# florasion/D-VQVAE

Measured on AMD Instinct MI355X. Metric: grasps/sec at batch=65536, N=1024 pts, K=512, higher is better.
Workload: dtype f32 (GEMMs: every fp32 operand as two fp16 pieces, a1 = fp16(a), a2 = fp16((a - a1) * 2^11), weights pre-scaled by one power of two per output row; the 3 partial products a1 b1, a1 b2, a2 b1 are exact in fp32 and accumulate in TWO fp32 accumulators (large / cross terms) on v_mfma_f32_16x16x32_f16; d

## Files before the change

d-vqvae_amd/csrc/gemm_f16x2.hip:

```cpp
#include "dvq_internal.h"
#include "gemm_common.h"

namespace {

typedef _Float16 h8 __attribute__((ext_vector_type(8)));
typedef _Float16 h2 __attribute__((ext_vector_type(2)));
typedef float f32x2 __attribute__((ext_vector_type(2)));

constexpr int TM = 128, TN = 256, BK = 32;
constexpr int A_PL = TM * 64;
constexpr int W_PL = TN * 64;
constexpr int STAGE = 2 * A_PL + 2 * W_PL;
constexpr float LO_SCALE = 1.0f / 2048.0f;

__device__ __forceinline__ int swz16(int row) { return (4 - ((row >> 2) & 3)) & 3; }

__device__ __forceinline__ void split2(const f32x4& lo, const f32x4& hi, h8& p1, h8& p2) {
    unsigned hb[4], lb[4];
    const float m2048 = -2048.0f;
#pragma unroll
    for (int j = 0; j < 4; ++j) {
        const float a0 = j < 2 ? lo[2 * j] : hi[2 * j - 4], a1 = j < 2 ? lo[2 * j + 1] : hi[2 * j - 3];
        hb[j] = __builtin_bit_cast(unsigned, __builtin_convertvector(f32x2{a0, a1}, h2));
        const float t0 = a0 * 2048.0f, t1 = a1 * 2048.0f;
        asm("v_fma_mixlo_f16 %0, %1, %2, %3 op_sel:[0,0,0] op_sel_hi:[1,0,0]" : "=v"(lb[j]) : "v"(hb[j]), "v"(m2048), "v"(t0));
        asm("v_fma_mixhi_f16 %0, %1, %2, %3 op_sel:[1,0,0] op_sel_hi:[1,0,0]" : "+v"(lb[j]) : "v"(hb[j]), "v"(m2048), "v"(t1));
    }
    p1 = __builtin_bit_cast(h8, uint4{hb[0], hb[1], hb[2], hb[3]});
    p2 = __builtin_bit_cast(h8, uint4{lb[0], lb[1], lb[2], lb[3]});
}

__device__ __forceinline__ f32x4 f16x2_combine(const f32x4& hi, const f32x4& lo, const float* ws, int n, bool vec) {
    f32x4 v = hi + lo * LO_SCALE;
    if (vec) v *= *reinterpret_cast<const f32x4*>(ws + n);
    return v;
}

__device__ __forceinline__ float relu_nan(float x) { return x < 0.f ? 0.f : x; }

template <int EPI>
__device__ __forceinline__ void f16x2_store_block(const GemmParams& p, long m, int n, f32x4 v, bool full) {
    if (full) {
        if (p.bias) v += *reinterpret_cast<const f32x4*>(p.bias + n);
        if constexpr (EPI == EPI_RESID) v += *reinterpret_cast<const f32x4*>(p.resid + m * p.ldr + n);
        if (p.relu) { v[0] = relu_nan(v[0]); v[1] = relu_nan(v[1]); v[2] = relu_nan(v[2]); v[3] = relu_nan(v[3]); }
        *reinterpret_cast<f32x4*>(p.out + m * p.ldo + n) = v;
    } else {
#pragma unroll
        for (int c = 0; c < 4; ++c) {
            if (n + c >= p.N) continue;
            float x = v[c] * p.wscale[n + c] + (p.bias ? p.bias[n + c] : 0.f);
            if constexpr (EPI == EPI_RESID) x += p.resid[m * p.ldr + n + c];
            if (p.relu) x = relu_nan(x);
            p.out[m * p.ldo + n + c] = x;
        }
    }
}

__device__ __forceinline__ float gate_act(float a, float g) {
    const float th = fmaf(-2.0f, __builtin_amdgcn_rcpf(1.0f + __builtin_amdgcn_exp2f(2.8853900817779268f * a)), 1.0f);
    const float sg = __builtin_amdgcn_rcpf(1.0f + __builtin_amdgcn_exp2f(-1.4426950408889634f * g));
    return th * sg;
}

__device__ __forceinline__ void f16x2_store_gate(const GemmParams& p, long m, int na, int c, f32x4 a, f32x4 g, const float* crow) {
    const int nb = na + 32;
    if (p.bias) {
        a += *reinterpret_cast<const f32x4*>(p.bias + na);
        g += *reinterpret_cast<const f32x4*>(p.bias + nb);
    }
    if (p.pre) {
        *reinterpret_cast<f32x4*>(p.pre + m * p.ldpre + na) = a;
        *reinterpret_cast<f32x4*>(p.pre + m * p.ldpre + nb) = g;
    }
    if (crow) {
        a += *reinterpret_cast<const f32x4*>(crow + na);
        g += *reinterpret_cast<const f32x4*>(crow + nb);
    }
    f32x4 o;
#pragma unroll
    for (int q = 0; q < 4; ++q) o[q] = gate_act(a[q], g[q]);
    *reinterpret_cast<f32x4*>(p.out + m * p.ldo + c) = o;
}

__device__ __forceinline__ f32x4 ld4(const float* q) { return *reinterpret_cast<const f32x4*>(q); }
__device__ __forceinline__ void st4(float* q, const f32x4& v) { *reinterpret_cast<f32x4*>(q) = v; }

template <int EPI, int NJ>
__device__ __forceinline__ void f16x2_epilogue_inside(const GemmParams& p, f32x4 (&hi)[NJ][4], f32x4 (&lo)[NJ][4], long m0w, int n0w, int c0w,
                                                      int lane) {
    static_assert(EPI == EPI_BIAS || EPI == EPI_RESID || (EPI == EPI_GATE && NJ == 4), "store epilogues with operands");
    const long m = m0w + (lane & 15);
    const int l4 = 4 * (lane >> 4), nl = n0w + l4;
    f32x4 ws[NJ], bq[NJ], aq[NJ][4];
    const float* crow[4];
#pragma unroll
    for (int jn = 0; jn < NJ; ++jn) ws[jn] = ld4(p.wscale + nl + 16 * jn);
    if (p.bias) {
#pragma unroll
        for (int jn = 0; jn < NJ; ++jn) bq[jn] = ld4(p.bias + nl + 16 * jn);
    }
    if constexpr (EPI == EPI_GATE) {
        if (p.cls) {
#pragma unroll
            for (int i = 0; i < 4; ++i) crow[i] = p.cls + (long)p.label[m + 16 * i] * p.N + nl;
        }
    }
#pragma unroll
    for (int jn = 0; jn < NJ; ++jn)
#pragma unroll
        for (int i = 0; i < 4; ++i) hi[jn][i] = hi[jn][i] + lo[jn][i] * LO_SCALE;
    if constexpr (EPI == EPI_RESID) {
#pragma unroll
        for (int i = 0; i < 4; ++i)
#pragma unroll
            for (int jn = 0; jn < NJ; ++jn) aq[jn][i] = ld4(p.resid + (m + 16 * i) * p.ldr + nl + 16 * jn);
    } else if constexpr (EPI == EPI_GATE) {
        if (p.cls) {
#pragma unroll
            for (int i = 0; i < 4; ++i)
#pragma unroll
                for (int jn = 0; jn < NJ; ++jn) aq[jn][i] = ld4(crow[i] + 16 * jn);
        }
    }
#pragma unroll
    for (int i = 0; i < 4; ++i) {
        if constexpr (EPI == EPI_GATE) {
#pragma unroll
            for (int jn = 0; jn < 2; ++jn) {
                f32x4 a = hi[jn][i] * ws[jn], g = hi[jn + 2][i] * ws[jn + 2];
                if (p.bias) { a += bq[jn]; g += bq[jn + 2]; }
                if (p.pre) {
                    st4(p.pre + (m + 16 * i) * p.ldpre + nl + 16 * jn, a);
                    st4(p.pre + (m + 16 * i) * p.ldpre + nl + 16 * jn + 32, g);
                }
                if (p.cls) { a += aq[jn][i]; g += aq[jn + 2][i]; }
                f32x4 o;
#pragma unroll
                for (int q = 0; q < 4; ++q) o[q] = gate_act(a[q], g[q]);
                st4(p.out + (m + 16 * i) * p.ldo + c0w + l4 + 16 * jn, o);
            }
        } else {
#pragma unroll
            for (int jn = 0; jn < NJ; ++jn) {
                f32x4 v = hi[jn][i] * ws[jn];
                if (p.bias) v += bq[jn];
                if constexpr (EPI == EPI_RESID) v += aq[jn][i];
                if (p.relu) { v[0] = relu_nan(v[0]); v[1] = relu_nan(v[1]); v[2] = relu_nan(v[2]); v[3] = relu_nan(v[3]); }
                st4(p.out + (m + 16 * i) * p.ldo + nl + 16 * jn, v);
            }
        }
    }
}

template <int NJ, bool INIT>
__device__ __forceinline__ void f16x2_init_acc(const GemmParams& p, f32x4 (&hi)[NJ][4], f32x4 (&lo)[NJ][4], long m0w, int n0w, int lane) {
    if constexpr (!INIT) {
#pragma unroll
        for (int a = 0; a < NJ; ++a)
#pragma unroll
            for (int c = 0; c < 4; ++c) { hi[a][c] = f32x4{0.f, 0.f, 0.f, 0.f}; lo[a][c] = f32x4{0.f, 0.f, 0.f, 0.f}; }
        return;
    }
    const int lr = lane & 15, lc = lane >> 4;
    if (p.acc_hi && m0w + 64 <= p.M && n0w + 16 * NJ <= p.N) {
        long r[4];
#pragma unroll
        for (int i = 0; i < 4; ++i) r[i] = m0w + i * 16 + lr;
        if (p.acc_row) {
#pragma unroll
            for (int i = 0; i < 4; ++i) r[i] = p.acc_row[r[i]];
        }
#pragma unroll
        for (int i = 0; i < 4; ++i)
#pragma unroll
            for (int jn = 0; jn < NJ; ++jn) {
                hi[jn][i] = ld4(p.acc_hi + r[i] * p.ldacc + n0w + jn * 16 + 4 * lc);
                lo[jn][i] = ld4(p.acc_lo + r[i] * p.ldacc + n0w + jn * 16 + 4 * lc);
            }
        return;
    }
#pragma unroll
    for (int i = 0; i < 4; ++i) {
        const long m = m0w + i * 16 + lr;
        const bool row_ok = p.acc_hi && m < p.M;
        const long r = row_ok ? (p.acc_row ? p.acc_row[m] : m) : 0;
#pragma unroll
        for (int jn = 0; jn < NJ; ++jn) {
            const int n = n0w + jn * 16 + 4 * lc;
            if (row_ok && n < p.N) {
                hi[jn][i] = *reinterpret_cast<const f32x4*>(p.acc_hi + r * p.ldacc + n);
                lo[jn][i] = *reinterpret_cast<const f32x4*>(p.acc_lo + r * p.ldacc + n);
            } else {
                hi[jn][i] = f32x4{0.f, 0.f, 0.f, 0.f};
                lo[jn][i] = f32x4{0.f, 0.f, 0.f, 0.f};
            }
        }
    }
}

template <int EPI, int NJ = 4>
__device__ __forceinline__ void f16x2_epilogue(const GemmParams& p, f32x4 (&hi)[NJ][4], f32x4 (&lo)[NJ][4], long m0w, int n0w, int c0w,
                                               int lane) {
    static_assert(NJ == 4 || EPI != EPI_GATE, "the gate pairs a wave's tanh columns with their partners 32 columns further");
    if constexpr (EPI == EPI_BIAS || EPI == EPI_RESID || (EPI == EPI_GATE && NJ == 4)) {
        const bool vec_ok = EPI == EPI_GATE || ((p.N % 4 == 0) && (p.ldo % 4 == 0) && (EPI != EPI_RESID || p.ldr % 4 == 0));
        if (vec_ok && m0w + 64 <= p.M && n0w + 16 * NJ <= p.N) {
            f16x2_epilogue_inside<EPI, NJ>(p, hi, lo, m0w, n0w, c0w, lane);
            return;
        }
    }
    const int lr = lane & 15, lc = lane >> 4;
#pragma unroll
    for (int i = 0; i < 4; ++i) {
        const long m = m0w + i * 16 + lr;
        if (m >= p.M) continue;
        if constexpr (EPI == EPI_BIAS || EPI == EPI_RESID) {
            const bool vec_ok = (p.N % 4 == 0) && (p.ldo % 4 == 0) && (EPI != EPI_RESID || p.ldr % 4 == 0);
#pragma unroll
            for (int jn = 0; jn < NJ; ++jn) {
                const int n = n0w + jn * 16 + 4 * lc;
                if (n >= p.N) continue;
                const bool full = vec_ok && n + 3 < p.N;
                f16x2_store_block<EPI>(p, m, n, f16x2_combine(hi[jn][i], lo[jn][i], p.wscale, n, full), full);
            }
        } else if constexpr (EPI == EPI_STATE) {
#pragma unroll
            for (int jn = 0; jn < NJ; ++jn) {
                const int n = n0w + jn * 16 + 4 * lc;
                if (n >= p.N) continue;
                *reinterpret_cast<f32x4*>(p.out + m * p.ldo + n) = hi[jn][i];
                *reinterpret_cast<f32x4*>(p.pre + m * p.ldpre + n) = lo[jn][i];
            }
        } else if constexpr (EPI == EPI_GATE) {
            if constexpr (NJ == 4) {
            if (n0w >= p.N) continue;
            const float* crow = p.cls ? p.cls + (long)p.label[m] * p.N : nullptr;
#pragma unroll
            for (int jn = 0; jn < 2; ++jn) {
                const int nl = jn * 16 + 4 * lc;
                const int na = n0w + nl;
                f16x2_store_gate(p, m, na, c0w + nl, f16x2_combine(hi[jn][i], lo[jn][i], p.wscale, na, true),
                                 f16x2_combine(hi[jn + 2][i], lo[jn + 2][i], p.wscale, na + 32, true), crow);
            }
            }
        }
    }
}

constexpr int PP_STAGES = 3;
constexpr size_t PP_SMEM = PP_STAGES * STAGE;
constexpr size_t PP_SMEM_N128 = PP_STAGES * (2 * A_PL + 2 * 128 * 64);

struct PpCursorA {
    int s, k_left;
    const float* a_ptr;
    __device__ __forceinline__ void open(const GemmParams& p, int src_i, long m0, int tid) {
        s = src_i;
        if (s >= p.nsrc) { k_left = 0; return; }
        const GemmSrc& src = p.src[s];
        k_left = src.K;
        long m = m0 + (tid >> 2);
        if (m >= p.M) m = p.M - 1;
        if (src.arow) m = src.arow[m];
        a_ptr = src.A + m * src.lda + 8 * (tid & 3);
    }
    __device__ __forceinline__ bool valid() const { return k_left > 0; }
    __device__ __forceinline__ void advance(const GemmParams& p, long m0, int tid) {
        a_ptr += BK;
        k_left -= BK;
        if (k_left <= 0) open(p, s + 1, m0, tid);
    }
};

template <int NJ>
struct PpCursorW {
    int s, k_left;
    const uint16_t* w_ptr[NJ];
    __device__ __forceinline__ void open(const GemmParams& p, int src_i, int n0, int wave, int lane) {
        s = src_i;
        if (s >= p.nsrc) { k_left = 0; return; }
        const GemmSrc& src = p.src[s];
        k_left = src.K;
#pragma unroll
        for (int i = 0; i < NJ; ++i) {
            const int id = wave * NJ + i;
            const int pl = id / (4 * NJ), rb = id % (4 * NJ);
            const int row = rb * 16 + (lane >> 2);
            int n = n0 + row;
            if (n >= p.N) n = p.N - 1;
            w_ptr[i] = src.Wp + pl * src.wp_plane + (long)n * src.ldw + 8 * ((lane & 3) ^ swz16(row));
        }
    }
    __device__ __forceinline__ void issue(char* stage, int wave) const {
#pragma unroll
        for (int i = 0; i < NJ; ++i) {
            const int id = wave * NJ + i;
            const int pl = id / (4 * NJ), rb = id % (4 * NJ);
            __builtin_amdgcn_global_load_lds((const __attribute__((address_space(1))) void*)w_ptr[i],
                                             (__attribute__((address_space(3))) void*)(stage + 2 * A_PL + pl * (64 * NJ * 64) + rb * 1024), 16, 0, 0);
        }
    }
    __device__ __forceinline__ void advance(const GemmParams& p, int n0, int wave, int lane) {
#pragma unroll
        for (int i = 0; i < NJ; ++i) w_ptr[i] += BK;
        k_left -= BK;
        if (k_left <= 0) open(p, s + 1, n0, wave, lane);
    }
};

template <int EPI, int NJ, bool INIT>
__global__ __launch_bounds__(512, 1) void gemm_f16x2_pp_kernel(const GemmParams p, int T) {
    extern __shared__ __attribute__((aligned(16))) char smem_c[];
    constexpr int TN = 64 * NJ, W_PL = TN * 64, STAGE = 2 * A_PL + 2 * W_PL;
    const int tid = threadIdx.x;
    const int tiles_n = (p.N + TN - 1) / TN;
    const long tiles_m = (p.M + TM - 1) / TM;
    const long b = blockIdx.x;
    const long j = b >> 3;
    const long mt = (j / tiles_n) * 8 + (b & 7);
    const int nt = (int)(j % tiles_n);
    if (mt >= tiles_m) return;
    const long m0 = mt * TM;
    const int n0 = nt * TN;
    const int lane = tid & 63;
    const int wave = __builtin_amdgcn_readfirstlane(tid >> 6);
    const int wm = wave >> 2, wn = wave & 3;

    PpCursorA ca;
    PpCursorW<NJ> cw;
    cw.open(p, 0, n0, wave, lane);
    const int a_dst = (tid >> 2) * 64 + 16 * ((tid & 3) ^ swz16(tid >> 2));
    f32x4 alo, ahi;
    auto load_a = [&](f32x4& qlo, f32x4& qhi) {
        qlo = *reinterpret_cast<const f32x4*>(ca.a_ptr);
        qhi = *reinterpret_cast<const f32x4*>(ca.a_ptr + 4);
        ca.advance(p, m0, tid);
    };
    auto store_a = [&](char* stage, const f32x4& qlo, const f32x4& qhi) {
        h8 p1, p2;
        split2(qlo, qhi, p1, p2);
        *reinterpret_cast<h8*>(stage + a_dst) = p1;
        *reinterpret_cast<h8*>(stage + A_PL + a_dst) = p2;
    };
    cw.issue(smem_c, wave);
    cw.advance(p, n0, wave, lane);
    if (T > 1) {
        cw.issue(smem_c + STAGE, wave);
        cw.advance(p, n0, wave, lane);
    }
    ca.open(p, 0, m0, tid);
    f32x4 a0lo, a0hi, a1lo, a1hi;
    load_a(a0lo, a0hi);
    if (T > 1) load_a(a1lo, a1hi);
    if (T > 2) load_a(alo, ahi);
    store_a(smem_c, a0lo, a0hi);
    if (T > 1) store_a(smem_c + STAGE, a1lo, a1hi);
    asm volatile("s_waitcnt vmcnt(0) lgkmcnt(0)" ::: "memory");
    __builtin_amdgcn_s_barrier();

    f32x4 hi[NJ][4], lo[NJ][4];
    f16x2_init_acc<NJ, INIT>(p, hi, lo, m0 + wm * 64, n0 + wn * 16 * NJ, lane);

    const int rd = (lane & 15) * 64 + 16 * ((lane >> 4) ^ swz16(lane & 15));
    if (wave >= 4) __builtin_amdgcn_s_barrier();
    int cur_st = 0, nx_st = 2;
    for (int t = 0; t < T; ++t) {
        const char* st = smem_c + cur_st * STAGE;
        h8 af[4][2], wf[NJ][2];
#pragma unroll
        for (int i = 0; i < 4; ++i)
#pragma unroll
            for (int pl = 0; pl < 2; ++pl) {
                if (DVQ_DIAG_ON && (p.dbg_abl & 128)) {
                    af[i][pl] = h8{};
                    if (i < NJ) wf[i][pl] = h8{};
                    continue;
                }
                if (DVQ_DIAG_ON && (p.dbg_abl & 64) && pl == 1) {
                    af[i][1] = af[i][0];
                    if (i < NJ) wf[i][1] = wf[i][0];
                    continue;
                }
                af[i][pl] = *reinterpret_cast<const h8*>(st + pl * A_PL + (wm * 64 + i * 16) * 64 + rd);
                if (i < NJ) wf[i][pl] = *reinterpret_cast<const h8*>(st + 2 * A_PL + pl * W_PL + (wn * 16 * NJ + i * 16) * 64 + rd);
            }
        asm volatile("s_waitcnt vmcnt(0)" ::: "memory");
        if (t + 2 < T) {
            char* nx = smem_c + nx_st * STAGE;
            if (!(DVQ_DIAG_ON && (p.dbg_abl & 16))) store_a(nx, alo, ahi);
            if (!(DVQ_DIAG_ON && (p.dbg_abl & 8))) cw.issue(nx, wave);
            cw.advance(p, n0, wave, lane);
            if (t + 3 < T && !(DVQ_DIAG_ON && (p.dbg_abl & 32))) load_a(alo, ahi);
        }
        asm volatile("s_waitcnt lgkmcnt(0)" ::: "memory");
        __builtin_amdgcn_s_barrier();
        __builtin_amdgcn_s_setprio(1);
        if (DVQ_DIAG_ON && (p.dbg_abl & 2)) {
#pragma unroll
            for (int i = 0; i < 4; ++i) asm volatile("" : : "v"(af[i][0]), "v"(af[i][1]), "v"(wf[i < NJ ? i : 0][0]), "v"(wf[i < NJ ? i : 0][1]));
        } else {
#pragma unroll
        for (int jn = 0; jn < NJ; ++jn)
#pragma unroll
            for (int i = 0; i < 4; ++i) hi[jn][i] = __builtin_amdgcn_mfma_f32_16x16x32_f16(wf[jn][0], af[i][0], hi[jn][i], 0, 0, 0);
#pragma unroll
        for (int jn = 0; jn < NJ; ++jn)
#pragma unroll
            for (int i = 0; i < 4; ++i) lo[jn][i] = __builtin_amdgcn_mfma_f32_16x16x32_f16(wf[jn][1], af[i][0], lo[jn][i], 0, 0, 0);
#pragma unroll
        for (int jn = 0; jn < NJ; ++jn)
#pragma unroll
            for (int i = 0; i < 4; ++i) lo[jn][i] = __builtin_amdgcn_mfma_f32_16x16x32_f16(wf[jn][0], af[i][1], lo[jn][i], 0, 0, 0);
        }
        __builtin_amdgcn_s_setprio(0);
        if (!(DVQ_DIAG_ON && (p.dbg_abl & 512))) __builtin_amdgcn_s_barrier();
        cur_st = cur_st == PP_STAGES - 1 ? 0 : cur_st + 1;
        nx_st = nx_st == PP_STAGES - 1 ? 0 : nx_st + 1;
    }
    if (wave < 4) __builtin_amdgcn_s_barrier();
    if (DVQ_DIAG_ON && (p.dbg_abl & 256)) {
        if (hi[0][0][0] + lo[0][0][0] == 12345.678f) p.out[0] = 1.f;
        return;
    }
    f16x2_epilogue<EPI, NJ>(p, hi, lo, m0 + wm * 64, n0 + wn * 16 * NJ, (n0 >> 1) + wn * 32, lane);
}

template <int EPI, int NJ, bool INIT>
int launch_pp(const GemmParams& p, hipStream_t stream) {
    constexpr size_t smem = NJ == 4 ? PP_SMEM : PP_SMEM_N128;
    static DvqOncePerDevice attr_once;
    DVQ_PROPAGATE(dvq_lds_limit(attr_once, reinterpret_cast<const void*>(&gemm_f16x2_pp_kernel<EPI, NJ, INIT>), smem, "gemm_f16x2"));
    const long grid = gemm_padded_grid((p.M + TM - 1) / TM, (p.N + 64 * NJ - 1) / (64 * NJ));
    const double ksum = gemm_ksum(p);
    {
        DVQ_PROF(gemm_prof_name(EPI, p.prof_cls), 2.0 * (double)p.M * p.N * ksum, ((double)p.M + p.N) * ksum * 4, stream);
        DVQ_LAUNCH((gemm_f16x2_pp_kernel<EPI, NJ, INIT>), dim3((unsigned)grid), dim3(512), smem, stream, p, gemm_ktiles(p, BK));
    }
    DVQ_CHECK_LAUNCH("gemm_f16x2");
    return DVQ_OK;
}

template <int EPI, bool INIT = false>
int launch_tiled(const GemmParams& p, hipStream_t stream) {
    if constexpr (EPI != EPI_GATE) {
        const long tiles_m = (p.M + TM - 1) / TM, tiles_n = (p.N + TN - 1) / TN, tiles_n2 = (p.N + 127) / 128, cus = dvq_num_cus();
        const long r256 = (tiles_m * tiles_n + cus - 1) / cus, r128 = (tiles_m * tiles_n2 + cus - 1) / cus;
        bool narrow = r128 < 2 * r256;
        if (dvq_knobs().gemm_tn == 128) narrow = true;
        if (dvq_knobs().gemm_tn == 256) narrow = false;
        if (narrow) return launch_pp<EPI, 2, INIT>(p, stream);
    }
    return launch_pp<EPI, 4, INIT>(p, stream);
}

template <int NB>
struct SkinnySlot {
    uint4 w[NB][2];
    f32x4 a[2];
};

template <int NB>
struct SkinnyCursor16 {
    int s, k_left;
    const float* a_ptr;
    const uint16_t* w_ptr[NB][2];

    __device__ __forceinline__ void open(const GemmParams& p, int src_i, long m, const int (&n)[NB], int lc) {
        s = src_i;
        const GemmSrc& src = p.src[s];
        k_left = src.K;
        a_ptr = src.A + (src.arow ? src.arow[m] : m) * src.lda + 8 * lc;
#pragma unroll
        for (int b = 0; b < NB; ++b)
#pragma unroll
            for (int pl = 0; pl < 2; ++pl) w_ptr[b][pl] = src.Wp + pl * src.wp_plane + (long)n[b] * src.ldw + 8 * lc;
    }
    __device__ __forceinline__ void load(SkinnySlot<NB>& t) const {
#pragma unroll
        for (int b = 0; b < NB; ++b) {
            t.w[b][0] = *reinterpret_cast<const uint4*>(w_ptr[b][0]);
            t.w[b][1] = *reinterpret_cast<const uint4*>(w_ptr[b][1]);
        }
        t.a[0] = *reinterpret_cast<const f32x4*>(a_ptr);
        t.a[1] = *reinterpret_cast<const f32x4*>(a_ptr + 4);
    }
    __device__ __forceinline__ void advance(const GemmParams& p, long m, const int (&n)[NB], int lc, bool last) {
        if (last) return;
        k_left -= BK;
        if (k_left > 0) {
            a_ptr += BK;
#pragma unroll
            for (int b = 0; b < NB; ++b) { w_ptr[b][0] += BK; w_ptr[b][1] += BK; }
        } else open(p, s + 1, m, n, lc);
    }
};

template <int EPI, int R>
__device__ __forceinline__ int skinny_col(int g, int j) {
    if constexpr (EPI == EPI_GATE) {
        constexpr int per64 = 32 / R;
        const int c0 = 64 * (g / per64) + R * (g % per64);
        return j < R ? c0 + j : (j < 2 * R ? c0 + 32 + (j - R) : c0);
    } else {
        return j < R ? R * g + j : R * g;
    }
}

template <int EPI, int R, int NB, int PF>
__device__ __forceinline__ void skinny_body(const GemmParams& p, int T, int groups) {
    const int lane = threadIdx.x;
    const int lr = lane & 15, lc = lane >> 4;
    const long mb0 = (long)blockIdx.y * 16;
    long m = mb0 + lr;
    if (m >= p.M) m = p.M - 1;
    int g[NB], n[NB];
#pragma unroll
    for (int b = 0; b < NB; ++b) {
        g[b] = (int)blockIdx.x * NB + b;
        if (g[b] >= groups) g[b] = groups - 1;
        n[b] = skinny_col<EPI, R>(g[b], lr);
        if (n[b] >= p.N) n[b] = p.N - 1;
    }
    f32x4 hi[NB], lo[NB];
#pragma unroll
    for (int b = 0; b < NB; ++b) {
        hi[b] = f32x4{0.f, 0.f, 0.f, 0.f};
        lo[b] = f32x4{0.f, 0.f, 0.f, 0.f};
        const int nc0 = skinny_col<EPI, R>(g[b], 4 * lc);
        const bool col_live = EPI == EPI_GATE ? 4 * lc < 2 * R : (4 * lc < R && nc0 < p.N);
        if (p.acc_hi && col_live && mb0 + lr < p.M) {
            const long r = p.acc_row ? p.acc_row[mb0 + lr] : mb0 + lr;
            hi[b] = *reinterpret_cast<const f32x4*>(p.acc_hi + r * p.ldacc + nc0);
            lo[b] = *reinterpret_cast<const f32x4*>(p.acc_lo + r * p.ldacc + nc0);
        }
    }
    SkinnyCursor16<NB> cur;
    cur.open(p, 0, m, n, lc);
    SkinnySlot<NB> slot[PF];
    int issued = 0;
#pragma unroll
    for (int u = 0; u < PF; ++u) {
        cur.load(slot[u]);
        cur.advance(p, m, n, lc, issued + 1 >= T);
        issued = issued + 1 < T ? issued + 1 : T;
    }
    for (int t = 0; t < T; t += PF) {
#pragma unroll
        for (int u = 0; u < PF; ++u) {
            if (t + u < T) {
                h8 a1, a2;
                split2(slot[u].a[0], slot[u].a[1], a1, a2);
#pragma unroll
                for (int b = 0; b < NB; ++b) {
                    const h8 w1 = __builtin_bit_cast(h8, slot[u].w[b][0]), w2 = __builtin_bit_cast(h8, slot[u].w[b][1]);
                    hi[b] = __builtin_amdgcn_mfma_f32_16x16x32_f16(w1, a1, hi[b], 0, 0, 0);
                    lo[b] = __builtin_amdgcn_mfma_f32_16x16x32_f16(w2, a1, lo[b], 0, 0, 0);
                    lo[b] = __builtin_amdgcn_mfma_f32_16x16x32_f16(w1, a2, lo[b], 0, 0, 0);
                }
            }
            cur.load(slot[u]);
            cur.advance(p, m, n, lc, issued + 1 >= T);
            issued = issued + 1 < T ? issued + 1 : T;
        }
    }
    const long mo = mb0 + lr;
#pragma unroll
    for (int b = 0; b < NB; ++b) {
        if (b > 0 && (int)blockIdx.x * NB + b >= groups) break;
        const int nc = skinny_col<EPI, R>(g[b], 4 * lc);
        if constexpr (EPI == EPI_GATE) {
            const bool live = 4 * lc < 2 * R && mo < p.M;
            f32x4 v = {0.f, 0.f, 0.f, 0.f};
            if (live) {
                v = f16x2_combine(hi[b], lo[b], p.wscale, nc, true);
                if (p.bias) v += *reinterpret_cast<const f32x4*>(p.bias + nc);
                if (p.pre) *reinterpret_cast<f32x4*>(p.pre + mo * p.ldpre + nc) = v;
                if (p.cls) v += *reinterpret_cast<const f32x4*>(p.cls + (long)p.label[mo] * p.N + nc);
            }
            f32x4 gg;
#pragma unroll
            for (int q = 0; q < 4; ++q) gg[q] = __shfl(v[q], lane + 4 * R, 64);
            if (live && 4 * lc < R) {
                f32x4 o;
#pragma unroll
                for (int q = 0; q < 4; ++q) o[q] = gate_act(v[q], gg[q]);
                const int c = 32 * (nc >> 6) + (nc & 31);
                *reinterpret_cast<f32x4*>(p.out + mo * p.ldo + c) = o;
            }
        } else if constexpr (EPI == EPI_STATE) {
            if (4 * lc >= R || mo >= p.M || nc >= p.N) continue;
            *reinterpret_cast<f32x4*>(p.out + mo * p.ldo + nc) = hi[b];
            *reinterpret_cast<f32x4*>(p.pre + mo * p.ldpre + nc) = lo[b];
        } else {
            if (4 * lc >= R || mo >= p.M || nc >= p.N) continue;
            const bool vec_ok = (p.N % 4 == 0) && (p.ldo % 4 == 0) && (EPI != EPI_RESID || p.ldr % 4 == 0);
            const bool full = vec_ok && nc + 3 < p.N;
            f16x2_store_block<EPI>(p, mo, nc, f16x2_combine(hi[b], lo[b], p.wscale, nc, full), full);
        }
    }
}

template <int EPI, int R, int NB, int PF>
__global__ __launch_bounds__(64) void gemm_f16x2_skinny_kernel(const GemmParams p, int T, int groups) {
    skinny_body<EPI, R, NB, PF>(p, T, groups);
}

struct GemmGroup {
    GemmParams p[DVQ_GEMM_GROUP_MAX];
    int T[DVQ_GEMM_GROUP_MAX];
};
template <int R, int NB, int PF>
__global__ __launch_bounds__(64) void gemm_f16x2_skinny_gate_group_kernel(const GemmGroup g, int groups) {
    skinny_body<EPI_GATE, R, NB, PF>(g.p[blockIdx.z], g.T[blockIdx.z], groups);
}

constexpr long SKINNY_MAX_M = 256;
inline long skinny_max_m(const GemmParams& p) { return p.prof_cls ? 4 * SKINNY_MAX_M : SKINNY_MAX_M; }

template <int EPI>
constexpr int skinny_cols = EPI == EPI_GATE ? 8 : 16;

template <int EPI>
int launch_skinny(const GemmParams& p, hipStream_t stream) {
    constexpr int R = skinny_cols<EPI>;
    const double ksum = gemm_ksum(p);
    const int T = gemm_ktiles(p, BK);
    const int gy = (int)((p.M + 15) / 16);
    const int groups = EPI == EPI_GATE ? (p.N / 64) * (32 / R) : (p.N + R - 1) / R;
    {
        DVQ_PROF(gemm_prof_name(EPI, p.prof_cls), 2.0 * (double)p.M * p.N * ksum, ((double)p.M + p.N) * ksum * 4, stream);
        if (gy >= 3) DVQ_LAUNCH((gemm_f16x2_skinny_kernel<EPI, R, 2, 4>), dim3((unsigned)((groups + 1) / 2), (unsigned)gy), dim3(64), 0, stream, p, T, groups);
        else DVQ_LAUNCH((gemm_f16x2_skinny_kernel<EPI, R, 1, 8>), dim3((unsigned)groups, (unsigned)gy), dim3(64), 0, stream, p, T, groups);
    }
    DVQ_CHECK_LAUNCH("gemm_f16x2_skinny");
    return DVQ_OK;
}

int launch_skinny_gate_group(const GemmParams* ps, int n, hipStream_t stream) {
    constexpr int R = skinny_cols<EPI_GATE>;
    GemmGroup g = {};
    double flops = 0, bytes = 0;
    for (int i = 0; i < n; ++i) {
        g.p[i] = ps[i];
        g.T[i] = gemm_ktiles(ps[i], BK);
        const double ksum = gemm_ksum(ps[i]);
        flops += 2.0 * (double)ps[i].M * ps[i].N * ksum;
        bytes += ((double)ps[i].M + ps[i].N) * ksum * 4;
    }
    const int gy = (int)((ps[0].M + 15) / 16);
    const int groups = (ps[0].N / 64) * (32 / R);
    {
        DVQ_PROF(gemm_prof_name(EPI_GATE, ps[0].prof_cls), flops, bytes, stream);
        if (gy >= 3) DVQ_LAUNCH((gemm_f16x2_skinny_gate_group_kernel<R, 2, 4>), dim3((unsigned)((groups + 1) / 2), (unsigned)gy, (unsigned)n), dim3(64), 0, stream, g, groups);
        else DVQ_LAUNCH((gemm_f16x2_skinny_gate_group_kernel<R, 1, 8>), dim3((unsigned)groups, (unsigned)gy, (unsigned)n), dim3(64), 0, stream, g, groups);
    }
    DVQ_CHECK_LAUNCH("gemm_f16x2_skinny_group");
    return DVQ_OK;
}

__global__ void f16x2_absmax_kernel(const float* __restrict__ w, long rows, int N, int K, float* __restrict__ absmax) {
    const long row = (long)blockIdx.x * (blockDim.x >> 6) + (threadIdx.x >> 6);
    if (row >= rows) return;
    const int lane = threadIdx.x & 63;
    const float* src = w + row * K;
    float mx = 0.f;
    for (int k = lane; k < K; k += 64) {
        const float v = fabsf(src[k]);
        mx = (v > mx || v != v) ? v : mx;
    }
#pragma unroll
    for (int o = 32; o > 0; o >>= 1) {
        const float ov = __shfl_xor(mx, o);
        mx = (ov > mx || ov != ov) ? ov : mx;
    }
    if (lane == 0) {
        atomicMax(reinterpret_cast<unsigned*>(absmax + row % N), __float_as_uint(mx));
    }
}

__device__ __forceinline__ int f16x2_exponent(float amax) {
    if (!(amax > 0.f) || !(amax < INFINITY)) return 0;
    int e;
    (void)frexpf(amax, &e);
    int t = 15 - e;
    if (t > 126) t = 126;
    if (t < -126) t = -126;
    return t;
}

__global__ void f16x2_split_kernel(const float* __restrict__ w, long total, int N, int K, const float* __restrict__ absmax,
                                   uint16_t* __restrict__ planes, float* __restrict__ row_scale) {
    const long i = (long)blockIdx.x * blockDim.x + threadIdx.x;
    if (i >= total) return;
    const int n = (int)((i / K) % N);
    const int t = f16x2_exponent(absmax[n]);
    const float ws = ldexpf(w[i], t);
    const _Float16 h1 = (_Float16)ws;
    const float r = ws - (float)h1;
    const _Float16 h2v = (_Float16)(r * 2048.0f);
    planes[i] = __builtin_bit_cast(uint16_t, h1);
    planes[total + i] = __builtin_bit_cast(uint16_t, h2v);
    if (i < N) row_scale[i] = ldexpf(1.0f, -f16x2_exponent(absmax[i]));
}

}

static int check_f16x2(const GemmParams& p, GemmEpilogue epi) {
    DVQ_REQUIRE(p.wscale, "gemm_f16x2: planes without row scales");
    for (int s = 0; s < p.nsrc; ++s) {
        const GemmSrc& g = p.src[s];
        DVQ_REQUIRE(g.Wp && dvq_aligned16(g.Wp) && g.wp_plane % 8 == 0 && g.ldw % 8 == 0, "gemm_f16x2: weight planes of source %d are not 16-byte aligned", s);
    }
    bool a_ok = true;
    for (int s = 0; s < p.nsrc; ++s) a_ok = a_ok && dvq_aligned16(p.src[s].A) && p.src[s].lda % 4 == 0;
    DVQ_REQUIRE(a_ok, "gemm_f16x2: activation rows are not 16-byte aligned");
    if (epi == EPI_GATE)
        DVQ_REQUIRE(dvq_aligned16(p.out) && p.ldo % 4 == 0 && (!p.pre || (dvq_aligned16(p.pre) && p.ldpre % 4 == 0)), "gemm_f16x2: gate outputs are not 16-byte aligned");
    if (epi == EPI_STATE)
        DVQ_REQUIRE(p.out && p.pre && dvq_aligned16(p.out) && dvq_aligned16(p.pre) && p.ldo % 4 == 0 && p.ldpre % 4 == 0 && p.N % 4 == 0,
                    "gemm_f16x2: accumulator-state outputs need N %% 4 == 0 and 16-byte aligned rows");
    if (p.acc_hi)
        DVQ_REQUIRE(epi == EPI_GATE && p.acc_lo && dvq_aligned16(p.acc_hi) && dvq_aligned16(p.acc_lo) && p.ldacc % 4 == 0 && p.N % 4 == 0,
                    "gemm_f16x2: an accumulator state needs both sums, N %% 4 == 0 and 16-byte aligned rows");
    return DVQ_OK;
}

int dvq_launch_gemm_f16x2_gate_group(const GemmParams* ps, int n, hipStream_t stream) {
    if (!dvq_knobs().gemm_skinny || ps[0].M > skinny_max_m(ps[0])) return -1;
    for (int i = 0; i < n; ++i) DVQ_PROPAGATE(check_f16x2(ps[i], EPI_GATE));
    return launch_skinny_gate_group(ps, n, stream);
}

int dvq_launch_gemm_f16x2(const GemmParams& p, GemmEpilogue epi, hipStream_t stream) {
    DVQ_PROPAGATE(check_f16x2(p, epi));
#ifdef DVQ_DIAG
    if (const char* e = getenv("DVQ_GEMM_ABL")) const_cast<GemmParams&>(p).dbg_abl = atoi(e);
#endif
    if (dvq_knobs().gemm_skinny && p.M <= skinny_max_m(p)) switch (epi) {
        case EPI_BIAS: return launch_skinny<EPI_BIAS>(p, stream);
        case EPI_RESID: return launch_skinny<EPI_RESID>(p, stream);
        case EPI_GATE: return launch_skinny<EPI_GATE>(p, stream);
        case EPI_STATE: return launch_skinny<EPI_STATE>(p, stream);
        default: break;
    }
    switch (epi) {
        case EPI_BIAS: return launch_tiled<EPI_BIAS>(p, stream);
        case EPI_RESID: return launch_tiled<EPI_RESID>(p, stream);
        case EPI_GATE: return p.acc_hi ? launch_tiled<EPI_GATE, true>(p, stream) : launch_tiled<EPI_GATE, false>(p, stream);
        case EPI_STATE: return launch_tiled<EPI_STATE>(p, stream);
        default: break;
    }
    dvq_set_error("gemm_f16x2: epilogue %d is not available on the fp16 split path", (int)epi);
    return DVQ_EINVAL;
}

extern "C" int dvq_f16x2_row_absmax(const float* w, int64_t outer, int N, int K, float* row_absmax, dvq_stream_t stream) {
    DVQ_REQUIRE(outer >= 1 && N >= 1 && K >= 1 && w && row_absmax, "f16x2_row_absmax: bad arguments");
    const long rows = (long)outer * N;
    DVQ_LAUNCH(f16x2_absmax_kernel, dim3((unsigned)((rows + 3) / 4)), dim3(256), 0, (hipStream_t)stream, w, rows, N, K, row_absmax);
    DVQ_CHECK_LAUNCH("f16x2_row_absmax");
    return DVQ_OK;
}

extern "C" int dvq_split_f16x2(const float* w, int64_t outer, int N, int K, const float* row_absmax, uint16_t* planes, float* row_scale,
                               dvq_stream_t stream) {
    DVQ_REQUIRE(outer >= 1 && N >= 1 && K >= 1 && w && row_absmax && planes && row_scale, "split_f16x2: bad arguments");
    const long total = (long)outer * N * K;
    DVQ_LAUNCH(f16x2_split_kernel, dim3((unsigned)((total + 255) / 256)), dim3(256), 0, (hipStream_t)stream, w, total, N, K, row_absmax, planes,
               row_scale);
    DVQ_CHECK_LAUNCH("split_f16x2");
    return DVQ_OK;
}
```

Baseline: 202,100.

## Peel GEMM pipeline tail and precompute cursor addresses for source switches

Restructures the triple-buffered fp16x2 GEMM main loop into a compile-time-specialised k-tile body: steady-state iterations with full prefetch, followed by peeled tail iterations. This removes the per-iteration `t+2<T` / `t+3<T` checks. The A and W cursors now count tiles and prefetch the next source's pointers, strides and row indices ahead of time, so switching between sources no longer reads GemmParams on the critical path. LDS addresses are precomputed as address-space-3 pointers with rotating stage offsets, and the barriers are fenced with sched_barrier. The aim is to cut scalar and address overhead and branch cost in the hot loop. The risk is higher register pressure, and the tile count now assumes K is a multiple of BK.

After: 208,300 (median of 6 runs). +3.1%, better.

```diff
diff --git a/d-vqvae_amd/csrc/gemm_f16x2.hip b/d-vqvae_amd/csrc/gemm_f16x2.hip
--- a/d-vqvae_amd/csrc/gemm_f16x2.hip
+++ b/d-vqvae_amd/csrc/gemm_f16x2.hip
@@ -252,60 +252,113 @@
 constexpr size_t PP_SMEM = PP_STAGES * STAGE;
 constexpr size_t PP_SMEM_N128 = PP_STAGES * (2 * A_PL + 2 * 128 * 64);
 
+typedef __attribute__((address_space(3))) char lds_char;
+typedef __attribute__((address_space(3))) h8 lds_h8;
+
+template <int V>
+struct PpConst { static constexpr int value = V; };
+
 struct PpCursorA {
-    int s, k_left;
+    int s, tiles;
     const float* a_ptr;
-    __device__ __forceinline__ void open(const GemmParams& p, int src_i, long m0, int tid) {
-        s = src_i;
-        if (s >= p.nsrc) { k_left = 0; return; }
-        const GemmSrc& src = p.src[s];
-        k_left = src.K;
-        long m = m0 + (tid >> 2);
+    const float* n_a;
+    long n_lda;
+    int n_k;
+    long n_row;
+    const int64_t* nn_arow;
+    __device__ __forceinline__ long row(const GemmParams& p, long m0, int tid) const {
+        const long m = m0 + (tid >> 2);
+        return m < p.M ? m : p.M - 1;
+    }
+    __device__ __forceinline__ void fetch(const GemmParams& p) {
+        const int i1 = min(s + 1, p.nsrc - 1), i2 = min(s + 2, p.nsrc - 1);
+        n_a = p.src[i1].A;
+        n_lda = p.src[i1].lda;
+        n_k = p.src[i1].K;
+        nn_arow = p.src[i2].arow;
+    }
+    __device__ __forceinline__ void open(const GemmParams& p, long m0, int tid) {
+        s = 0;
+        const GemmSrc& src = p.src[0];
+        const long m = row(p, m0, tid);
+        const int64_t* arow1 = p.src[min(1, p.nsrc - 1)].arow;
+        const long r0 = src.arow ? src.arow[m] : m;
+        n_row = arow1 ? arow1[m] : m;
+        tiles = (int)((unsigned)src.K / BK);
+        a_ptr = src.A + r0 * src.lda + 8 * (tid & 3);
+        fetch(p);
+    }
+    __device__ __forceinline__ void next_source(const GemmParams& p, long m0, int tid) {
+        asm volatile("" : "+v"(tid));
+        a_ptr = n_a + n_row * n_lda + 8 * (tid & 3);
+        tiles = (int)((unsigned)n_k / BK);
+        ++s;
+        int q = tid >> 2;
+        asm volatile("" : "+v"(q) : "v"(a_ptr));
+        long m = m0 + q;
         if (m >= p.M) m = p.M - 1;
-        if (src.arow) m = src.arow[m];
-        a_ptr = src.A + m * src.lda + 8 * (tid & 3);
-    }
-    __device__ __forceinline__ bool valid() const { return k_left > 0; }
-    __device__ __forceinline__ void advance(const GemmParams& p, long m0, int tid) {
+        n_row = nn_arow ? nn_arow[m] : m;
+    }
+    __device__ __forceinline__ bool advance(const GemmParams& p, long m0, int tid) {
         a_ptr += BK;
-        k_left -= BK;
-        if (k_left <= 0) open(p, s + 1, m0, tid);
+        if (__builtin_expect(--tiles != 0, 1)) return false;
+        next_source(p, m0, tid);
+        return true;
     }
 };
 
 template <int NJ>
 struct PpCursorW {
-    int s, k_left;
+    int s, tiles;
+    lds_char* dma_dst[NJ];
     const uint16_t* w_ptr[NJ];
-    __device__ __forceinline__ void open(const GemmParams& p, int src_i, int n0, int wave, int lane) {
-        s = src_i;
-        if (s >= p.nsrc) { k_left = 0; return; }
-        const GemmSrc& src = p.src[s];
-        k_left = src.K;
+    const uint16_t* n_wp;
+    long n_plane, n_ldw;
+    int n_k;
+    __device__ __forceinline__ void fetch(const GemmParams& p) {
+        const int i1 = min(s + 1, p.nsrc - 1);
+        n_wp = p.src[i1].Wp;
+        n_plane = p.src[i1].wp_plane;
+        n_ldw = p.src[i1].ldw;
+        n_k = p.src[i1].K;
+    }
+    __device__ __forceinline__ void place(const GemmParams& p, const uint16_t* wp, long plane, long ldw, int n0, int wave, int lane) {
+        const uint16_t* base = wp + (wave >> 2) * plane + 8 * ((lane & 3) ^ swz16(lane >> 2));
+        const int nr = n0 + (wave & 3) * (16 * NJ) + (lane >> 2);
+#pragma unroll
+        for (int i = 0; i < NJ; ++i) w_ptr[i] = base + (long)min(nr + 16 * i, p.N - 1) * ldw;
+    }
+    __device__ __forceinline__ void open(const GemmParams& p, int n0, int wave, int lane) {
+        s = 0;
+        const GemmSrc& src = p.src[0];
+        tiles = (int)((unsigned)src.K / BK);
+        place(p, src.Wp, src.wp_plane, src.ldw, n0, wave, lane);
+        fetch(p);
+    }
+    __device__ __forceinline__ void set_wave(const char* smem, int wave) {
 #pragma unroll
         for (int i = 0; i < NJ; ++i) {
             const int id = wave * NJ + i;
             const int pl = id / (4 * NJ), rb = id % (4 * NJ);
-            const int row = rb * 16 + (lane >> 2);
-            int n = n0 + row;
-            if (n >= p.N) n = p.N - 1;
-            w_ptr[i] = src.Wp + pl * src.wp_plane + (long)n * src.ldw + 8 * ((lane & 3) ^ swz16(row));
-        }
-    }
-    __device__ __forceinline__ void issue(char* stage, int wave) const {
-#pragma unroll
-        for (int i = 0; i < NJ; ++i) {
-            const int id = wave * NJ + i;
-            const int pl = id / (4 * NJ), rb = id % (4 * NJ);
+            dma_dst[i] = (lds_char*)smem + (2 * A_PL + pl * (64 * NJ * 64) + rb * 1024);
+            asm volatile("" : "+s"(dma_dst[i]));
+        }
+    }
+    __device__ __forceinline__ void issue(int stage_off) const {
+#pragma unroll
+        for (int i = 0; i < NJ; ++i)
             __builtin_amdgcn_global_load_lds((const __attribute__((address_space(1))) void*)w_ptr[i],
-                                             (__attribute__((address_space(3))) void*)(stage + 2 * A_PL + pl * (64 * NJ * 64) + rb * 1024), 16, 0, 0);
-        }
-    }
-    __device__ __forceinline__ void advance(const GemmParams& p, int n0, int wave, int lane) {
+                                             (__attribute__((address_space(3))) void*)(dma_dst[i] + stage_off), 16, 0, 0);
+    }
+    __device__ __forceinline__ bool advance(const GemmParams& p, int n0, int wave, int lane) {
 #pragma unroll
         for (int i = 0; i < NJ; ++i) w_ptr[i] += BK;
-        k_left -= BK;
-        if (k_left <= 0) open(p, s + 1, n0, wave, lane);
+        if (__builtin_expect(--tiles != 0, 1)) return false;
+        asm volatile("" : "+v"(lane));
+        place(p, n_wp, n_plane, n_ldw, n0, wave, lane);
+        tiles = (int)((unsigned)n_k / BK);
+        ++s;
+        return true;
     }
 };
 
@@ -329,33 +382,54 @@
 
     PpCursorA ca;
     PpCursorW<NJ> cw;
-    cw.open(p, 0, n0, wave, lane);
+    int refetch = 0;
+    auto fetch_next = [&]() {
+        if (refetch & 1) cw.fetch(p);
+        if (refetch & 2) ca.fetch(p);
+        refetch = 0;
+    };
+    cw.open(p, n0, wave, lane);
+    cw.set_wave(smem_c, wave);
     const int a_dst = (tid >> 2) * 64 + 16 * ((tid & 3) ^ swz16(tid >> 2));
     f32x4 alo, ahi;
     auto load_a = [&](f32x4& qlo, f32x4& qhi) {
         qlo = *reinterpret_cast<const f32x4*>(ca.a_ptr);
         qhi = *reinterpret_cast<const f32x4*>(ca.a_ptr + 4);
-        ca.advance(p, m0, tid);
+        if (ca.advance(p, m0, tid)) refetch |= 2;
     };
-    auto store_a = [&](char* stage, const f32x4& qlo, const f32x4& qhi) {
+    auto step_w = [&]() {
+        if (cw.advance(p, n0, wave, lane)) refetch |= 1;
+    };
+    auto store_a = [&](lds_char* dst, const f32x4& qlo, const f32x4& qhi) {
         h8 p1, p2;
         split2(qlo, qhi, p1, p2);
-        *reinterpret_cast<h8*>(stage + a_dst) = p1;
-        *reinterpret_cast<h8*>(stage + A_PL + a_dst) = p2;
+        *reinterpret_cast<lds_h8*>(dst) = p1;
+        *reinterpret_cast<lds_h8*>(dst + A_PL) = p2;
     };
-    cw.issue(smem_c, wave);
-    cw.advance(p, n0, wave, lane);
+    char* const st0 = smem_c;
+    char* const st1 = smem_c + STAGE;
+    cw.issue(0);
+    step_w();
+    if (refetch) fetch_next();
     if (T > 1) {
-        cw.issue(smem_c + STAGE, wave);
-        cw.advance(p, n0, wave, lane);
-    }
-    ca.open(p, 0, m0, tid);
+        cw.issue(STAGE);
+        step_w();
+        if (refetch) fetch_next();
+    }
+    ca.open(p, m0, tid);
     f32x4 a0lo, a0hi, a1lo, a1hi;
     load_a(a0lo, a0hi);
-    if (T > 1) load_a(a1lo, a1hi);
-    if (T > 2) load_a(alo, ahi);
-    store_a(smem_c, a0lo, a0hi);
-    if (T > 1) store_a(smem_c + STAGE, a1lo, a1hi);
+    if (refetch) fetch_next();
+    if (T > 1) {
+        load_a(a1lo, a1hi);
+        if (refetch) fetch_next();
+    }
+    if (T > 2) {
+        load_a(alo, ahi);
+        if (refetch) fetch_next();
+    }
+    store_a((lds_char*)st0 + a_dst, a0lo, a0hi);
+    if (T > 1) store_a((lds_char*)st1 + a_dst, a1lo, a1hi);
     asm volatile("s_waitcnt vmcnt(0) lgkmcnt(0)" ::: "memory");
     __builtin_amdgcn_s_barrier();
 
@@ -363,10 +437,22 @@
     f16x2_init_acc<NJ, INIT>(p, hi, lo, m0 + wm * 64, n0 + wn * 16 * NJ, lane);
 
     const int rd = (lane & 15) * 64 + 16 * ((lane >> 4) ^ swz16(lane & 15));
+    lds_char* fr_a = (lds_char*)smem_c + (wm * 64 * 64 + rd);
+    lds_char* fr_w = (lds_char*)smem_c + (2 * A_PL + wn * 16 * NJ * 64 + rd);
+    lds_char* wr_a = (lds_char*)smem_c + a_dst;
+    asm volatile("" : "+v"(fr_a), "+v"(fr_w), "+v"(wr_a));
+    int st_cur = 0, st_n1 = STAGE, st_nx = 2 * STAGE;
     if (wave >= 4) __builtin_amdgcn_s_barrier();
-    int cur_st = 0, nx_st = 2;
-    for (int t = 0; t < T; ++t) {
-        const char* st = smem_c + cur_st * STAGE;
+    auto phase_barrier = [&]() __attribute__((always_inline)) {
+        __builtin_amdgcn_sched_barrier(0);
+        __builtin_amdgcn_s_barrier();
+        __builtin_amdgcn_sched_barrier(0);
+    };
+    auto ktile = [&](auto feed_c) __attribute__((always_inline)) {
+        constexpr int FEED = decltype(feed_c)::value;
+        if (!(DVQ_DIAG_ON && (p.dbg_abl & 512))) phase_barrier();
+        const lds_char* const st_a = fr_a + st_cur;
+        const lds_char* const st_w = fr_w + st_cur;
         h8 af[4][2], wf[NJ][2];
 #pragma unroll
         for (int i = 0; i < 4; ++i)
@@ -382,19 +468,21 @@
                     if (i < NJ) wf[i][1] = wf[i][0];
                     continue;
                 }
-                af[i][pl] = *reinterpret_cast<const h8*>(st + pl * A_PL + (wm * 64 + i * 16) * 64 + rd);
-                if (i < NJ) wf[i][pl] = *reinterpret_cast<const h8*>(st + 2 * A_PL + pl * W_PL + (wn * 16 * NJ + i * 16) * 64 + rd);
-            }
-        asm volatile("s_waitcnt vmcnt(0)" ::: "memory");
-        if (t + 2 < T) {
-            char* nx = smem_c + nx_st * STAGE;
-            if (!(DVQ_DIAG_ON && (p.dbg_abl & 16))) store_a(nx, alo, ahi);
-            if (!(DVQ_DIAG_ON && (p.dbg_abl & 8))) cw.issue(nx, wave);
-            cw.advance(p, n0, wave, lane);
-            if (t + 3 < T && !(DVQ_DIAG_ON && (p.dbg_abl & 32))) load_a(alo, ahi);
+                af[i][pl] = *reinterpret_cast<const lds_h8*>(st_a + pl * A_PL + i * 16 * 64);
+                if (i < NJ) wf[i][pl] = *reinterpret_cast<const lds_h8*>(st_w + pl * W_PL + i * 16 * 64);
+            }
+        if constexpr (FEED >= 1) asm volatile("s_waitcnt vmcnt(0)" : "+v"(alo), "+v"(ahi) : : "memory");
+        else asm volatile("s_waitcnt vmcnt(0)" ::: "memory");
+        if constexpr (FEED >= 1) {
+            if (!(DVQ_DIAG_ON && (p.dbg_abl & 16))) store_a(wr_a + st_nx, alo, ahi);
+            if (!(DVQ_DIAG_ON && (p.dbg_abl & 8))) cw.issue(st_nx);
+            if constexpr (FEED == 2) {
+                step_w();
+                if (!(DVQ_DIAG_ON && (p.dbg_abl & 32))) load_a(alo, ahi);
+            }
         }
         asm volatile("s_waitcnt lgkmcnt(0)" ::: "memory");
-        __builtin_amdgcn_s_barrier();
+        phase_barrier();
         __builtin_amdgcn_s_setprio(1);
         if (DVQ_DIAG_ON && (p.dbg_abl & 2)) {
 #pragma unroll
@@ -413,11 +501,19 @@
 #pragma unroll
             for (int i = 0; i < 4; ++i) lo[jn][i] = __builtin_amdgcn_mfma_f32_16x16x32_f16(wf[jn][0], af[i][1], lo[jn][i], 0, 0, 0);
         }
+        if constexpr (FEED == 2) {
+            if (__builtin_expect(refetch != 0, 0)) fetch_next();
+        }
+        const int st_free = st_cur;
+        st_cur = st_n1;
+        st_n1 = st_nx;
+        st_nx = st_free;
         __builtin_amdgcn_s_setprio(0);
-        if (!(DVQ_DIAG_ON && (p.dbg_abl & 512))) __builtin_amdgcn_s_barrier();
-        cur_st = cur_st == PP_STAGES - 1 ? 0 : cur_st + 1;
-        nx_st = nx_st == PP_STAGES - 1 ? 0 : nx_st + 1;
-    }
+    };
+    for (int t = 3; t < T; ++t) ktile(PpConst<2>{});
+    if (T > 2) ktile(PpConst<1>{});
+    if (T > 1) ktile(PpConst<0>{});
+    ktile(PpConst<0>{});
     if (wave < 4) __builtin_amdgcn_s_barrier();
     if (DVQ_DIAG_ON && (p.dbg_abl & 256)) {
         if (hi[0][0][0] + lo[0][0][0] == 12345.678f) p.out[0] = 1.f;
```
